# ilovin/lstm_ctc_ocr

Hardware: NVIDIA H100
Metric: text-line images/sec (fwd+CTC loss) (higher is better)
Workload: dtype bf16

## Files before the change

### lstm_ctc_ocr_b200/csrc/lstm.cuh

```cuda
#pragma once
#include <cuda.h>

#include "common.cuh"
#include "wgmma.cuh"

namespace lstm {

constexpr int NUM_THREADS = 384;
constexpr int BLOCK_M = 128;

struct Params {
  const __nv_bfloat16* xproj;
  __nv_bfloat16* h_state;
  __nv_bfloat16* lstm_out;
  const int* seq_len;
  int Nimg, Npad, H, T, tiles_per_dir;
  __nv_bfloat16* gates;
  float* csave;
  int swap_ls;
  long long* trace;
};

#define LSTM_TRACE(ev)                                                                                  \
  do {                                                                                                  \
    if (p.trace != nullptr && lane == 0 && s >= 8 && s < 12 && (blockIdx.x == 0 || blockIdx.x == 5))    \
      p.trace[(((blockIdx.x ? 1 : 0) * 4 + (s - 8)) * 16) + (ev)] = clock64();                          \
  } while (0)

__device__ __forceinline__ uint32_t cluster_ctarank() {
  uint32_t r;
  asm volatile("mov.u32 %0, %%cluster_ctarank;" : "=r"(r));
  return r;
}
__device__ __forceinline__ void cluster_arrive_release() { asm volatile("barrier.cluster.arrive.release.aligned;" ::: "memory"); }
__device__ __forceinline__ void cluster_wait_acquire() { asm volatile("barrier.cluster.wait.acquire.aligned;" ::: "memory"); }
__device__ __forceinline__ void fence_proxy_async_all() { asm volatile("fence.proxy.async;" ::: "memory"); }

template <int CS>
struct Cfg {
  static constexpr int UPC = 256 / CS;
  static constexpr int NCOLS = 4 * UPC;
  static constexpr int B_BYTES = 4 * NCOLS * 128;
  static constexpr int A_BYTES = 4 * BLOCK_M * 128;
  static constexpr int ACC_OFFSET = A_BYTES + B_BYTES;
  static constexpr int BAR_OFFSET = ACC_OFFSET + BLOCK_M * NCOLS * 4;
  static constexpr int SMEM_BYTES = BAR_OFFSET + 128 + 1024;
};

template <int CS>
__global__ void __launch_bounds__(NUM_THREADS, 1)
lstm_persistent_kernel(const __grid_constant__ CUtensorMap tmH, const __grid_constant__ CUtensorMap tmW, const Params p) {
  static_assert(CS == 8, "register budget of the epilogue is sized for 32 units per CTA");
  using C = Cfg<CS>;
  constexpr int UPC = C::UPC, NCOLS = C::NCOLS;
  constexpr int HALF = UPC / 2;

  extern __shared__ uint8_t smem_raw[];
  uint8_t* smem = reinterpret_cast<uint8_t*>((reinterpret_cast<uintptr_t>(smem_raw) + 1023) & ~uintptr_t(1023));
  uint8_t* smem_a = smem;
  uint8_t* smem_b = smem + C::A_BYTES;
  uint64_t* a_full = reinterpret_cast<uint64_t*>(smem + C::BAR_OFFSET);
  uint64_t* b_full = a_full + 4;
  float* acc_tile = reinterpret_cast<float*>(smem + C::ACC_OFFSET);

  const int warp_idx = threadIdx.x >> 5, lane = threadIdx.x & 31;
  const int rank = (int)cluster_ctarank();
  const int unit = blockIdx.x / CS;
  const int dir = unit / p.tiles_per_dir;
  const int tile = unit - dir * p.tiles_per_dir;

  if (warp_idx == 0 && lane == 0) {
    ptx::prefetch_tmap(&tmH);
    ptx::prefetch_tmap(&tmW);
    for (int i = 0; i < 4; ++i) ptx::mbar_init(&a_full[i], 1);
    ptx::mbar_init(b_full, 1);
    ptx::fence_barrier_init();
  }
  __syncthreads();

  if (warp_idx == 0 && lane == 0) {
// ... 98 lines not shown
          if (p.gates != nullptr) {
            const size_t dts = (size_t)unit * p.T + s;
            __nv_bfloat16* gs = p.gates + lstm_gate_off(dts, 0, rank * UPC + u0, row);
            float* cs = p.csave + lstm_c_off(dts, rank * UPC + u0, row);
#pragma unroll
            for (int i = 0; i < HALF; i += 8) {
              *reinterpret_cast<uint4*>(gs + 0 * LSTM_GATE_STRIDE + (i >> 3) * LSTM_GCHUNK_STRIDE) = make_uint4(ptx::pack_bf16x2(__uint_as_float(gi[i]), __uint_as_float(gi[i + 1])), ptx::pack_bf16x2(__uint_as_float(gi[i + 2]), __uint_as_float(gi[i + 3])), ptx::pack_bf16x2(__uint_as_float(gi[i + 4]), __uint_as_float(gi[i + 5])), ptx::pack_bf16x2(__uint_as_float(gi[i + 6]), __uint_as_float(gi[i + 7])));
              *reinterpret_cast<uint4*>(gs + 1 * LSTM_GATE_STRIDE + (i >> 3) * LSTM_GCHUNK_STRIDE) = make_uint4(ptx::pack_bf16x2(__uint_as_float(gj[i]), __uint_as_float(gj[i + 1])), ptx::pack_bf16x2(__uint_as_float(gj[i + 2]), __uint_as_float(gj[i + 3])), ptx::pack_bf16x2(__uint_as_float(gj[i + 4]), __uint_as_float(gj[i + 5])), ptx::pack_bf16x2(__uint_as_float(gj[i + 6]), __uint_as_float(gj[i + 7])));
              *reinterpret_cast<uint4*>(gs + 2 * LSTM_GATE_STRIDE + (i >> 3) * LSTM_GCHUNK_STRIDE) = make_uint4(ptx::pack_bf16x2(__uint_as_float(gf[i]), __uint_as_float(gf[i + 1])), ptx::pack_bf16x2(__uint_as_float(gf[i + 2]), __uint_as_float(gf[i + 3])), ptx::pack_bf16x2(__uint_as_float(gf[i + 4]), __uint_as_float(gf[i + 5])), ptx::pack_bf16x2(__uint_as_float(gf[i + 6]), __uint_as_float(gf[i + 7])));
              *reinterpret_cast<uint4*>(gs + 3 * LSTM_GATE_STRIDE + (i >> 3) * LSTM_GCHUNK_STRIDE) = make_uint4(ptx::pack_bf16x2(__uint_as_float(go[i]), __uint_as_float(go[i + 1])), ptx::pack_bf16x2(__uint_as_float(go[i + 2]), __uint_as_float(go[i + 3])), ptx::pack_bf16x2(__uint_as_float(go[i + 4]), __uint_as_float(go[i + 5])), ptx::pack_bf16x2(__uint_as_float(go[i + 6]), __uint_as_float(go[i + 7])));
            }
#pragma unroll
            for (int i = 0; i < HALF; i += 4)
              *reinterpret_cast<float4*>(cs + (i >> 2) * LSTM_CCHUNK_STRIDE) = make_float4(cst[u0 + i], cst[u0 + i + 1], cst[u0 + i + 2], cst[u0 + i + 3]);
          }
#pragma unroll
          for (int i = 0; i < HALF / 2; ++i) hp[i] = ptx::pack_bf16x2(hv[2 * i], hv[2 * i + 1]);
        } else {
#pragma unroll
          for (int i = 0; i < HALF / 2; ++i) hp[i] = 0u;
        }
        if (okn) {
#pragma unroll
          for (int i = 0; i < HALF / 2; i += 4) {
            const uint4 v = make_uint4(hp[i], hp[i + 1], hp[i + 2], hp[i + 3]);
            *reinterpret_cast<uint4*>(hn + u0 + 2 * i) = v;
            *reinterpret_cast<uint4*>(lo + u0 + 2 * i) = v;
          }
        }
      }
      if (warp_idx == 4) LSTM_TRACE(8);
      fence_proxy_async_all();
      if (warp_idx == 4) LSTM_TRACE(9);
    }
    cluster_arrive_release();
    if (warp_idx == 4) LSTM_TRACE(10);
    cluster_wait_acquire();
    if (warp_idx == 4) LSTM_TRACE(11);
  }
}


template <int EW>
struct McThreads {
  static constexpr int EPI = EW * 32;
  static constexpr int ALL = 128 + EPI;
};

template <int CS>
struct CfgMc {
  static constexpr int UPC = 256 / CS;
  static constexpr int NCOLS = 4 * UPC;
  static constexpr int B_BYTES = 4 * NCOLS * 128;
  static constexpr int A_BYTES = 32 * BLOCK_M * 16;
  static constexpr int SLICE_BYTES = A_BYTES / CS;
  static constexpr int ACC_OFFSET = 2 * A_BYTES + B_BYTES;
  static constexpr int BAR_OFFSET = ACC_OFFSET + BLOCK_M * 64 * 4;
  static constexpr int SMEM_BYTES = BAR_OFFSET + 128 + 1024;
};

__device__ __forceinline__ void bulk_copy_s2s_cluster(uint32_t dst_cluster_addr, const void* src_smem, uint32_t bytes,
                                                      uint32_t bar_cluster_addr) {
  asm volatile("cp.async.bulk.shared::cluster.shared::cta.mbarrier::complete_tx::bytes [%0], [%1], %2, [%3];" ::"r"(dst_cluster_addr),
               "r"(ptx::smem_u32(src_smem)), "r"(bytes), "r"(bar_cluster_addr)
               : "memory");
}

template <int CS, int MODE, int EW>
__global__ void __launch_bounds__(McThreads<EW>::ALL, 1)
lstm_mc_kernel(const __grid_constant__ CUtensorMap tmW, const Params p) {
  static_assert(CS == 8, "8 CTAs x 32 units");
  using C = CfgMc<CS>;
  constexpr int UPC = C::UPC, NCOLS = C::NCOLS;
  constexpr int HALF = UPC / (EW / 4);
  constexpr int MC_EPI_THREADS = McThreads<EW>::EPI;
  static_assert(EW == 8, "epilogue warps = the two MMA warpgroups");
  constexpr bool DS = (MODE == 1), MS = (MODE == 2), GX = (MODE == 3), LOCAL = DS || MS;
  constexpr uint32_t FILL_TX = LOCAL ? (CS - 1) * C::SLICE_BYTES : C::A_BYTES;

  extern __shared__ uint8_t smem_raw[];
  uint8_t* smem = smem_raw + ((1024u - (ptx::smem_u32(smem_raw) & 1023u)) & 1023u);
  uint8_t* smem_a = smem;
  uint8_t* smem_b = smem + 2 * C::A_BYTES;
  uint64_t* a_full = reinterpret_cast<uint64_t*>(smem + C::BAR_OFFSET);
  uint64_t* b_full = a_full + 2;
  uint64_t* part_ready = b_full + 1;
  float* acc_half = reinterpret_cast<float*>(smem + C::ACC_OFFSET);

  const int warp_idx = threadIdx.x >> 5, lane = threadIdx.x & 31;
  const int rank = (int)cluster_ctarank();
  const int unit = blockIdx.x / CS;
  const int dir = unit / p.tiles_per_dir;
  const int tile = unit - dir * p.tiles_per_dir;

  if (warp_idx == 0 && lane == 0) {
    ptx::prefetch_tmap(&tmW);
    ptx::mbar_init(&part_ready[0], CS);
    ptx::mbar_init(&part_ready[1], CS);
    ptx::mbar_init(&a_full[0], GX ? MC_EPI_THREADS : LOCAL ? 2 : 1);
    ptx::mbar_init(&a_full[1], GX ? MC_EPI_THREADS : LOCAL ? 2 : 1);
    ptx::mbar_init(b_full, 1);
    ptx::fence_barrier_init();
    if (!GX && p.T > 1) ptx::mbar_arrive_expect_tx(&a_full[1], FILL_TX);
    if (!GX && p.T > 2) ptx::mbar_arrive_expect_tx(&a_full[0], FILL_TX);
    ptx::mbar_arrive_expect_tx(b_full, C::B_BYTES);
    for (int kb = 0; kb < 4; ++kb)
      ptx::tma_load_2d(&tmW, b_full, smem_b + kb * NCOLS * 128, kb * 64, dir * 1024 + rank * NCOLS);
  }
  __syncthreads();
  cluster_arrive_release();
  cluster_wait_acquire();

  if (warp_idx < 4) {
    ptx::setmaxnreg_dec<40>();
  } else {
    ptx::setmaxnreg_inc<232>();
    const int wgi = (warp_idx >> 2) - 1;
    const int q = warp_idx & 3;
    const int hh = (warp_idx - 4) >> 2;
    const int u0 = hh * HALF;
    const int row = q * 32 + lane;
    const int n = tile * BLOCK_M + row;
    const bool okn = n < p.Nimg;
    const int len = okn ? min(max(__ldg(p.seq_len + n), 0), p.T) : 0;
    float cst[HALF];
#pragma unroll
    for (int i = 0; i < HALF; ++i) cst[i] = 0.f;
    ptx::mbar_wait(b_full, 0);
    const uint32_t slice_off = rank * C::SLICE_BYTES + (u0 / 8) * 2048 + row * 16;
    uint8_t* hx0 = reinterpret_cast<uint8_t*>(p.h_state) + ((size_t)unit * CS + rank) * C::SLICE_BYTES;
    const size_t hx_buf_stride = (size_t)2 * p.tiles_per_dir * CS * C::SLICE_BYTES;

    for (int s = 0; s < p.T; ++s) {
      const bool active = s < len;
      const int t = active ? (dir ? (len - 1 - s) : s) : s;
      uint4 xp[4][HALF / 8];
      if (active) {
        const __nv_bfloat16* src = p.xproj + ((size_t)n * p.H + s) * 2048 + dir * 1024 + rank * NCOLS + u0;
#pragma unroll
        for (int g = 0; g < 4; ++g)
#pragma unroll
          for (int v = 0; v < HALF / 8; ++v) xp[g][v] = __ldg(reinterpret_cast<const uint4*>(src + g * UPC) + v);
      }
      if (warp_idx == 4) LSTM_TRACE(5);
      uint32_t gi[HALF], gj[HALF], gf[HALF], go[HALF];
      if (s > 0) {
        const int b = s & 1;
        ptx::mbar_wait(&a_full[b], ((s - 1) >> 1) & 1);
        if (warp_idx == 4) LSTM_TRACE(3);
        if (!GX && s + 2 < p.T && threadIdx.x == 128) ptx::mbar_arrive_expect_tx(&a_full[b], FILL_TX);
        const uint32_t a_base = ptx::smem_u32(smem_a + b * C::A_BYTES) + wgi * 64 * 16;
        float d[NCOLS / 2];
        wg::fence();
#pragma unroll
        for (int k = 0; k < 16; ++k) {
          const uint64_t a_desc = p.swap_ls ? ptx::make_desc_k_nosw(a_base + k * 4096, 128, 2048) : ptx::make_desc_k_nosw(a_base + k * 4096, 2048, 128);
          const uint64_t b_desc = ptx::make_desc_k_sw128(ptx::smem_u32(smem_b + (k >> 2) * NCOLS * 128)) + 2 * (k & 3);
          wg::mma_bf16<NCOLS>(d, a_desc, b_desc, k != 0);
        }
        wg::commit();
        wg::wait<0>();
        wg::fence_operand(d);
        if (warp_idx == 4) LSTM_TRACE(4);
        const int tt = threadIdx.x & 127, l = tt & 31;
        const int r0 = wgi * 64 + 16 * (tt >> 5) + (l >> 2);
#pragma unroll
        for (int r = 0; r < 2; ++r) {
          ptx::bar_sync(1, MC_EPI_THREADS);
#pragma unroll
          for (int g = 0; g < 4; ++g)
#pragma unroll
            for (int jj = 0; jj < 2; ++jj) {
              const int j = 4 * g + 2 * r + jj;
              const int c = g * 16 + jj * 8 + 2 * (l & 3);
              *reinterpret_cast<float2*>(ptx::acc_chunk<64>(acc_half, r0, c >> 2) + (c & 3)) = make_float2(d[4 * j], d[4 * j + 1]);
              *reinterpret_cast<float2*>(ptx::acc_chunk<64>(acc_half, r0 + 8, c >> 2) + (c & 3)) = make_float2(d[4 * j + 2], d[4 * j + 3]);
            }
          ptx::bar_sync(1, MC_EPI_THREADS);
          if (hh == r) {
            ptx::acc_ld<64, HALF>(acc_half, row, 0, gi);
            ptx::acc_ld<64, HALF>(acc_half, row, 16, gj);
            ptx::acc_ld<64, HALF>(acc_half, row, 32, gf);
            ptx::acc_ld<64, HALF>(acc_half, row, 48, go);
          }
        }
        if (warp_idx == 4) LSTM_TRACE(7);
      } else {
#pragma unroll
        for (int i = 0; i < HALF; ++i) { gi[i] = 0u; gj[i] = 0u; gf[i] = 0u; go[i] = 0u; }
      }
      uint32_t hp[HALF / 2];
      if (active) {
        const uint32_t* xi = reinterpret_cast<const uint32_t*>(xp[0]);
        const uint32_t* xj = reinterpret_cast<const uint32_t*>(xp[1]);
        const uint32_t* xf = reinterpret_cast<const uint32_t*>(xp[2]);
        const uint32_t* xo = reinterpret_cast<const uint32_t*>(xp[3]);
        float hv[HALF];
#pragma unroll
        for (int i = 0; i < HALF; ++i) {
          const float zi = __uint_as_float(gi[i]) + ((i & 1) ? ptx::bf16_hi(xi[i >> 1]) : ptx::bf16_lo(xi[i >> 1]));
          const float zj = __uint_as_float(gj[i]) + ((i & 1) ? ptx::bf16_hi(xj[i >> 1]) : ptx::bf16_lo(xj[i >> 1]));
          const float zf = __uint_as_float(gf[i]) + ((i & 1) ? ptx::bf16_hi(xf[i >> 1]) : ptx::bf16_lo(xf[i >> 1]));
          const float zo = __uint_as_float(go[i]) + ((i & 1) ? ptx::bf16_hi(xo[i >> 1]) : ptx::bf16_lo(xo[i >> 1]));
          const float ai = ptx::fast_sigmoid(zi), aj = ptx::fast_tanh(zj), af = ptx::fast_sigmoid(zf), ao = ptx::fast_sigmoid(zo);
          const float c = af * cst[i] + ai * aj;
          cst[i] = c;
          hv[i] = ao * ptx::fast_tanh(c);
          if (p.gates != nullptr) {
            gi[i] = __float_as_uint(ai); gj[i] = __float_as_uint(aj); gf[i] = __float_as_uint(af); go[i] = __float_as_uint(ao);
          }
        }
#pragma unroll
        for (int i = 0; i < HALF / 2; ++i) hp[i] = ptx::pack_bf16x2(hv[2 * i], hv[2 * i + 1]);
      } else {
#pragma unroll
        for (int i = 0; i < HALF / 2; ++i) hp[i] = 0u;
      }
      if (s + 1 < p.T) {
        const int nb = (s + 1) & 1;
        if (LOCAL) {
          uint8_t* dst = smem_a + nb * C::A_BYTES + slice_off;
#pragma unroll
          for (int v = 0; v < HALF / 8; ++v)
            *reinterpret_cast<uint4*>(dst + v * 2048) = make_uint4(hp[4 * v], hp[4 * v + 1], hp[4 * v + 2], hp[4 * v + 3]);
          ptx::fence_proxy_async_smem();
        } else {
          uint8_t* dst = hx0 + (size_t)nb * hx_buf_stride + (u0 / 8) * 2048 + row * 16;
#pragma unroll
          for (int v = 0; v < HALF / 8; ++v)
            *reinterpret_cast<uint4*>(dst + v * 2048) = make_uint4(hp[4 * v], hp[4 * v + 1], hp[4 * v + 2], hp[4 * v + 3]);
          if (!GX) fence_proxy_async_all();
        }
        if (warp_idx == 4) LSTM_TRACE(8);
        asm volatile("bar.sync 1, %0;" ::"n"(MC_EPI_THREADS) : "memory");
        if (warp_idx == 4) {
          uint8_t* my_slice = smem_a + nb * C::A_BYTES + rank * C::SLICE_BYTES;
          if (DS) {
            if (lane < CS) {
              if (lane == rank) {
                ptx::mbar_arrive(&a_full[nb]);
              } else {
                const uint32_t dst = ptx::mapa(ptx::smem_u32(my_slice), (uint32_t)lane);
                const uint32_t bar = ptx::mapa(ptx::smem_u32(&a_full[nb]), (uint32_t)lane);
                bulk_copy_s2s_cluster(dst, my_slice, C::SLICE_BYTES, bar);
              }
            }
          } else if (MS) {
            if (lane == 0) {
              uint8_t* g = hx0 + (size_t)nb * hx_buf_stride;
              ptx::bulk_store_1d(g, my_slice, C::SLICE_BYTES);
              ptx::bulk_commit();
              asm volatile("cp.async.bulk.wait_group 0;" ::: "memory");
              ptx::bulk_load_1d_mc(my_slice, g, C::SLICE_BYTES, &a_full[nb], (uint16_t)(((1u << CS) - 1) & ~(1u << rank)));
              ptx::mbar_arrive(&a_full[nb]);
            }
          } else if (GX) {
            if (lane < CS) ptx::mbar_arrive_cluster(ptx::mapa(ptx::smem_u32(&part_ready[nb]), (uint32_t)lane));
          } else if (lane == 0) {
            ptx::bulk_load_1d_mc(my_slice, hx0 + (size_t)nb * hx_buf_stride, C::SLICE_BYTES, &a_full[nb], (uint16_t)((1u << CS) - 1));
          }
          __syncwarp();
          LSTM_TRACE(9);
        }
        if (GX) {
          ptx::mbar_wait_cluster(&part_ready[nb], (uint32_t)(s >> 1) & 1u);
          const uint8_t* g = reinterpret_cast<const uint8_t*>(p.h_state) + (size_t)nb * hx_buf_stride + (size_t)unit * CS * C::SLICE_BYTES;
          uint8_t* d = smem_a + nb * C::A_BYTES;
          const int et = threadIdx.x - 128;
          uint4 v[C::A_BYTES / 16 / MC_EPI_THREADS];
#pragma unroll
          for (int k = 0; k < C::A_BYTES / 16 / MC_EPI_THREADS; ++k) v[k] = __ldcg(reinterpret_cast<const uint4*>(g) + k * MC_EPI_THREADS + et);
#pragma unroll
          for (int k = 0; k < C::A_BYTES / 16 / MC_EPI_THREADS; ++k) *(reinterpret_cast<uint4*>(d) + k * MC_EPI_THREADS + et) = v[k];
          ptx::fence_proxy_async_smem();
          ptx::mbar_arrive(&a_full[nb]);
        }
      }
      if (okn) {
        __nv_bfloat16* lo = p.lstm_out + ((size_t)n * p.H + t) * 512 + dir * 256 + rank * UPC + u0;
        if constexpr (HALF == 16) ptx::st_global_v8(lo, hp[0], hp[1], hp[2], hp[3], hp[4], hp[5], hp[6], hp[7]);
        else *reinterpret_cast<uint4*>(lo) = make_uint4(hp[0], hp[1], hp[2], hp[3]);
      }
      if (active && p.gates != nullptr) {
        const size_t dts = (size_t)unit * p.T + s;
        __nv_bfloat16* gs = p.gates + lstm_gate_off(dts, 0, rank * UPC + u0, row);
        float* cs = p.csave + lstm_c_off(dts, rank * UPC + u0, row);
#pragma unroll
        for (int i = 0; i < HALF; i += 8) {
          *reinterpret_cast<uint4*>(gs + 0 * LSTM_GATE_STRIDE + (i >> 3) * LSTM_GCHUNK_STRIDE) = make_uint4(ptx::pack_bf16x2(__uint_as_float(gi[i]), __uint_as_float(gi[i + 1])), ptx::pack_bf16x2(__uint_as_float(gi[i + 2]), __uint_as_float(gi[i + 3])), ptx::pack_bf16x2(__uint_as_float(gi[i + 4]), __uint_as_float(gi[i + 5])), ptx::pack_bf16x2(__uint_as_float(gi[i + 6]), __uint_as_float(gi[i + 7])));
          *reinterpret_cast<uint4*>(gs + 1 * LSTM_GATE_STRIDE + (i >> 3) * LSTM_GCHUNK_STRIDE) = make_uint4(ptx::pack_bf16x2(__uint_as_float(gj[i]), __uint_as_float(gj[i + 1])), ptx::pack_bf16x2(__uint_as_float(gj[i + 2]), __uint_as_float(gj[i + 3])), ptx::pack_bf16x2(__uint_as_float(gj[i + 4]), __uint_as_float(gj[i + 5])), ptx::pack_bf16x2(__uint_as_float(gj[i + 6]), __uint_as_float(gj[i + 7])));
          *reinterpret_cast<uint4*>(gs + 2 * LSTM_GATE_STRIDE + (i >> 3) * LSTM_GCHUNK_STRIDE) = make_uint4(ptx::pack_bf16x2(__uint_as_float(gf[i]), __uint_as_float(gf[i + 1])), ptx::pack_bf16x2(__uint_as_float(gf[i + 2]), __uint_as_float(gf[i + 3])), ptx::pack_bf16x2(__uint_as_float(gf[i + 4]), __uint_as_float(gf[i + 5])), ptx::pack_bf16x2(__uint_as_float(gf[i + 6]), __uint_as_float(gf[i + 7])));
          *reinterpret_cast<uint4*>(gs + 3 * LSTM_GATE_STRIDE + (i >> 3) * LSTM_GCHUNK_STRIDE) = make_uint4(ptx::pack_bf16x2(__uint_as_float(go[i]), __uint_as_float(go[i + 1])), ptx::pack_bf16x2(__uint_as_float(go[i + 2]), __uint_as_float(go[i + 3])), ptx::pack_bf16x2(__uint_as_float(go[i + 4]), __uint_as_float(go[i + 5])), ptx::pack_bf16x2(__uint_as_float(go[i + 6]), __uint_as_float(go[i + 7])));
        }
#pragma unroll
        for (int i = 0; i < HALF; i += 4) *reinterpret_cast<float4*>(cs + (i >> 2) * LSTM_CCHUNK_STRIDE) = make_float4(cst[i], cst[i + 1], cst[i + 2], cst[i + 3]);
      }
      if (warp_idx == 4) LSTM_TRACE(10);
    }
  }

  __syncthreads();
  cluster_arrive_release();
  cluster_wait_acquire();
}

}
```

### lstm_ctc_ocr_b200/csrc/model.cu

```cuda
#include <cstdarg>
#include <cstring>
#include <string>
#include <vector>

#include <cstdlib>
#include <condition_variable>
#include <mutex>
#include <thread>

#include "gemm_launch.h"
#include "lstm.cuh"
#include "conv_swap.cuh"
#include "conv1_tc.cuh"
#include "kernels.cuh"
#include "model_internal.h"

static thread_local char g_err[1024] = "";
int crnn_fail(int status, const char* fmt, ...) {
  va_list ap;
  va_start(ap, fmt);
  vsnprintf(g_err, sizeof(g_err), fmt, ap);
  va_end(ap);
  return status;
}
// ... 565 lines not shown
    float* bn = pl.bn;
    if (m->dp_world > 1)
      CRNN_TRY(dp_allreduce_bn_finalize(m, pl.stats, bn_count * m->dp_world, m->P("conv4_1/conv4_1/gamma"), m->P("conv4_1/conv4_1/beta"),
                                        m->cfg.bn_eps, bn, st));
    else
    CRNN_TRY(launch_bn_finalize(pl.stats, bn_count, m->P("conv4_1/conv4_1/gamma"), m->P("conv4_1/conv4_1/beta"),
                                m->cfg.bn_eps, bn, bn + 512, bn + 1024, bn + 1536, 512, st));
    CRNN_TRY(launch_bn_apply_relu(pl.a4a_pre, pl.a4a, bn, bn + 512, (size_t)N * H2 * 4, 512, st));
  }
  STAGE_MARK();
  {
    gemm::Params p = conv_params(N, H2, 4, 512, 512, 256, m->P("conv4_2/biases"), pl.a4b_pre, pl.mg4);
    p.stats = pl.stats + 1024;
    CRNN_TRY((launch_gemm<256, gemm::A_CONV3, gemm::EPI_STATS, 4>(pl.tA_c42, m->tB_c42, p, sms, st, &pl.tO_c42)));
    STAGE_MARK();
    float* bn = pl.bn + 2048;
    if (m->dp_world > 1)
      CRNN_TRY(dp_allreduce_bn_finalize(m, pl.stats + 1024, bn_count * m->dp_world, m->P("conv4_2/conv4_2/gamma"),
                                        m->P("conv4_2/conv4_2/beta"), m->cfg.bn_eps, bn, st));
    else
    CRNN_TRY(launch_bn_finalize(pl.stats + 1024, bn_count, m->P("conv4_2/conv4_2/gamma"), m->P("conv4_2/conv4_2/beta"),
                                m->cfg.bn_eps, bn, bn + 512, bn + 1024, bn + 1536, 512, st));
    CRNN_TRY(launch_bn_apply_relu_pool12(pl.a4b_pre, pl.a4b, bn, bn + 512, (size_t)N * H2 * 2, 512, st));
  }
  STAGE_MARK();
  {
    gemm::Params p;
    memset(&p, 0, sizeof(p));
    p.M = N * H2;
    p.num_m_tiles = (p.M + 127) / 128; p.num_n_tiles = 2; p.num_k_blocks = 32; p.kb_per_shift = 16; p.row_shift_mul = 1;
    p.Nc = 512; p.bias = m->P("conv5/biases"); p.out = pl.a5; p.ldo = 512;
    CRNN_TRY((launch_gemm<256, gemm::A_PLAIN, gemm::EPI_BIAS_BF16, 4>(pl.tA_c5, m->tB_c5, p, sms, st, &pl.tA_x)));
  }
  STAGE_MARK();
  {
    gemm::Params p;
    memset(&p, 0, sizeof(p));
    p.M = N * H2;
    p.num_m_tiles = (p.M + 127) / 128; p.num_n_tiles = 8; p.num_k_blocks = 8; p.kb_per_shift = 8;
    p.Nc = 2048; p.bias = m->xbias; p.out = pl.xproj; p.ldo = 2048;
    p.H = H2; p.T = T; p.seq_len = time_step_len;
    if (m->lstm_upc == 32) CRNN_TRY((launch_gemm<256, gemm::A_PLAIN, gemm::EPI_XPROJ, 4>(pl.tA_x, m->tB_x, p, sms, st, &pl.tO_x)));
    else CRNN_TRY((launch_gemm<256, gemm::A_PLAIN, gemm::EPI_BIAS_BF16, 4>(pl.tA_x, m->tB_x, p, sms, st, &pl.tO_x)));
  }
  STAGE_MARK();
  if (m->lstm_upc == 32) {
    constexpr int CS = 8;
    lstm::Params lp;
    lp.xproj = pl.xproj; lp.h_state = pl.h_state; lp.lstm_out = pl.lstm_out; lp.seq_len = time_step_len;
    lp.Nimg = N; lp.Npad = pl.Npad; lp.H = H2; lp.T = T; lp.tiles_per_dir = pl.Npad / 128;
    lp.gates = pl.train ? pl.gates : nullptr; lp.csave = pl.train ? pl.csave : nullptr;
    static long long* d_trace = nullptr;
    const bool want_trace = getenv("CRNN_LSTM_TRACE") != nullptr;
    if (want_trace && d_trace == nullptr) CUDA_TRY(cudaMalloc(&d_trace, 2 * 4 * 16 * sizeof(long long)));
    if (want_trace) CUDA_TRY(cudaMemsetAsync(d_trace, 0, 2 * 4 * 16 * sizeof(long long), st));
    lp.trace = want_trace ? d_trace : nullptr;
    lp.swap_ls = getenv("CRNN_LSTM_SWAPLS") != nullptr;
    auto kern = lstm::lstm_persistent_kernel<CS>;
    auto kern_mc = lstm::lstm_mc_kernel<CS, 0, 8>;
    auto kern_ds = lstm::lstm_mc_kernel<CS, 1, 8>;
    auto kern_ms = lstm::lstm_mc_kernel<CS, 2, 8>;
    auto kern_gx = lstm::lstm_mc_kernel<CS, 3, 8>;
    static bool attr = false;
    if (!attr) {
      CUDA_TRY(cudaFuncSetAttribute(kern, cudaFuncAttributeMaxDynamicSharedMemorySize, lstm::Cfg<CS>::SMEM_BYTES));
      CUDA_TRY(cudaFuncSetAttribute(kern_mc, cudaFuncAttributeMaxDynamicSharedMemorySize, lstm::CfgMc<CS>::SMEM_BYTES));
      CUDA_TRY(cudaFuncSetAttribute(kern_ds, cudaFuncAttributeMaxDynamicSharedMemorySize, lstm::CfgMc<CS>::SMEM_BYTES));
      CUDA_TRY(cudaFuncSetAttribute(kern_ms, cudaFuncAttributeMaxDynamicSharedMemorySize, lstm::CfgMc<CS>::SMEM_BYTES));
      CUDA_TRY(cudaFuncSetAttribute(kern_gx, cudaFuncAttributeMaxDynamicSharedMemorySize, lstm::CfgMc<CS>::SMEM_BYTES));
      attr = true;
    }
    cudaLaunchConfig_t cfg;
    memset(&cfg, 0, sizeof(cfg));
    cfg.gridDim = dim3(CS * 2 * lp.tiles_per_dir);
    cfg.blockDim = dim3(m->lstm_mc ? lstm::McThreads<8>::ALL : lstm::NUM_THREADS);
    cfg.dynamicSmemBytes = m->lstm_mc ? lstm::CfgMc<CS>::SMEM_BYTES : lstm::Cfg<CS>::SMEM_BYTES;
    cfg.stream = st;
    cudaLaunchAttribute at[1];
    at[0].id = cudaLaunchAttributeClusterDimension;
    at[0].val.clusterDim.x = CS; at[0].val.clusterDim.y = 1; at[0].val.clusterDim.z = 1;
    cfg.attrs = at; cfg.numAttrs = 1;
    if (m->lstm_mc == 4) CUDA_TRY(cudaLaunchKernelEx(&cfg, kern_gx, m->tB_h128, lp));
    else if (m->lstm_mc == 3) CUDA_TRY(cudaLaunchKernelEx(&cfg, kern_ms, m->tB_h128, lp));
    else if (m->lstm_mc == 2) CUDA_TRY(cudaLaunchKernelEx(&cfg, kern_ds, m->tB_h128, lp));
    else if (m->lstm_mc == 1) CUDA_TRY(cudaLaunchKernelEx(&cfg, kern_mc, m->tB_h128, lp));
    else CUDA_TRY(cudaLaunchKernelEx(&cfg, kern, pl.tA_hall, m->tB_h128, lp));
    if (want_trace) {
      long long h[2 * 4 * 16];
      CUDA_TRY(cudaStreamSynchronize(st));
      CUDA_TRY(cudaMemcpy(h, d_trace, sizeof(h), cudaMemcpyDeviceToHost));
      for (int c = 0; c < 2; ++c)
        for (int s = 0; s < 4; ++s) {
          fprintf(stderr, "lstm_trace cta%d step%d:", c ? 5 : 0, 8 + s);
          for (int e = 0; e < 12; ++e) fprintf(stderr, " %lld", h[(c * 4 + s) * 16 + e] ? h[(c * 4 + s) * 16 + e] - h[(c * 4) * 16] : -1);
          fprintf(stderr, "\n");
        }
    }
  } else {
    CUDA_TRY(cudaMemsetAsync(pl.h_state, 0, (size_t)2 * pl.Npad * 256 * 2, st));
    CUDA_TRY(cudaMemsetAsync(pl.c_state, 0, (size_t)2 * pl.Npad * 256 * 4, st));
    for (int s = 0; s < T; ++s) {
      gemm::Params p;
      memset(&p, 0, sizeof(p));
      p.num_m_tiles = 2 * pl.Npad / 128; p.num_n_tiles = 4; p.num_k_blocks = 4; p.kb_per_shift = 4;
      p.m_tiles_per_dir = pl.Npad / 128;
      p.Nc = 1024; p.H = H2; p.T = T; p.Nimg = N; p.Npad = pl.Npad; p.step = s;
      p.xproj = pl.xproj; p.c_state = pl.c_state; p.lstm_out = pl.lstm_out; p.seq_len = time_step_len;
      p.h_next = pl.h_state + (size_t)((s + 1) & 1) * 2 * pl.Npad * 256;
      CRNN_TRY((launch_gemm<256, gemm::A_PLAIN, gemm::EPI_LSTM, 4>(pl.tA_h[s & 1], m->tB_h, p, sms, st)));
    }
  }
  STAGE_MARK();
  {
    gemm::Params p;
    memset(&p, 0, sizeof(p));
    p.M = N * H2;
    p.num_m_tiles = (p.M + 127) / 128; p.num_n_tiles = 1; p.num_k_blocks = 8; p.kb_per_shift = 8;
    p.Nc = 64; p.bias = m->P("logits/biases"); p.out = logits_out; p.H = H2; p.T = T; p.Nimg = N;
    CRNN_TRY((launch_gemm<64, gemm::A_PLAIN, gemm::EPI_LOGITS, 8>(pl.tA_l, m->tB_l, p, sms, st)));
  }
  STAGE_MARK();
#undef STAGE_MARK
  return CRNN_OK;
}

extern "C" int crnn_forward(crnn_model* m, const float* data, const int* time_step_len, int N, int W, float* logits_out,
                            void* workspace, size_t workspace_bytes, crnn_stream_t stream) {
  cudaStream_t st = reinterpret_cast<cudaStream_t>(stream);
  return forward_impl(m, data, nullptr, time_step_len, N, W, logits_out, workspace, workspace_bytes, 1, st, st);
}

extern "C" int crnn_forward_host(crnn_model* m, const float* host_data, float* data_staging, const int* time_step_len, int N, int W,
                                 float* logits_out, void* workspace, size_t workspace_bytes, int chunks, crnn_stream_t stream,
                                 crnn_stream_t copy_stream) {
  if (!host_data || !data_staging) return crnn_fail(CRNN_INVALID_VALUE, "forward_host: null pointer");
  return forward_impl(m, data_staging, host_data, time_step_len, N, W, logits_out, workspace, workspace_bytes, chunks,
                      reinterpret_cast<cudaStream_t>(stream), reinterpret_cast<cudaStream_t>(copy_stream));
}

extern "C" int crnn_host_copy(void* dst, const void* src, size_t bytes, int threads) {
  if ((!dst || !src) && bytes) return crnn_fail(CRNN_INVALID_VALUE, "host_copy: null pointer");
  CopyPool::get().copy(dst, src, bytes, threads < 1 ? 1 : threads);
  return CRNN_OK;
}

extern "C" int crnn_forward_pageable(crnn_model* m, const float* pageable_data, float* pinned_staging, float* data_staging,
                                     const int* time_step_len, int N, int W, float* logits_out, void* workspace, size_t workspace_bytes,
                                     int chunks, int host_threads, crnn_stream_t stream, crnn_stream_t copy_stream) {
  if (!pageable_data || !pinned_staging || !data_staging) return crnn_fail(CRNN_INVALID_VALUE, "forward_pageable: null pointer");
// ... 139 lines not shown
```

Baseline: 173,200.

## Run LSTM cell math on WGMMA fragments in registers and decouple warpgroup halves

```diff
diff --git a/lstm_ctc_ocr_b200/csrc/lstm.cuh b/lstm_ctc_ocr_b200/csrc/lstm.cuh
--- a/lstm_ctc_ocr_b200/csrc/lstm.cuh
+++ b/lstm_ctc_ocr_b200/csrc/lstm.cuh
@@ -21,11 +21,12 @@
   long long* trace;
 };
 
-#define LSTM_TRACE(ev)                                                                                  \
+#define LSTM_TRACE_WG(wg, ev)                                                                           \
   do {                                                                                                  \
     if (p.trace != nullptr && lane == 0 && s >= 8 && s < 12 && (blockIdx.x == 0 || blockIdx.x == 5))    \
-      p.trace[(((blockIdx.x ? 1 : 0) * 4 + (s - 8)) * 16) + (ev)] = clock64();                          \
+      p.trace[((((blockIdx.x ? 1 : 0) * 2 + (wg)) * 4 + (s - 8)) * 16) + (ev)] = clock64();             \
   } while (0)
+#define LSTM_TRACE(ev) LSTM_TRACE_WG(0, ev)
 
 __device__ __forceinline__ uint32_t cluster_ctarank() {
   uint32_t r;
@@ -230,10 +231,11 @@
   static constexpr int UPC = 256 / CS;
   static constexpr int NCOLS = 4 * UPC;
   static constexpr int B_BYTES = 4 * NCOLS * 128;
-  static constexpr int A_BYTES = 32 * BLOCK_M * 16;
-  static constexpr int SLICE_BYTES = A_BYTES / CS;
-  static constexpr int ACC_OFFSET = 2 * A_BYTES + B_BYTES;
-  static constexpr int BAR_OFFSET = ACC_OFFSET + BLOCK_M * 64 * 4;
+  static constexpr int HALF_ROWS = BLOCK_M / 2;
+  static constexpr int HALF_A_BYTES = 32 * HALF_ROWS * 16;
+  static constexpr int A_BYTES = 2 * HALF_A_BYTES;
+  static constexpr int SLICE_BYTES = HALF_A_BYTES / CS;
+  static constexpr int BAR_OFFSET = 2 * A_BYTES + B_BYTES;
   static constexpr int SMEM_BYTES = BAR_OFFSET + 128 + 1024;
 };
 
@@ -250,20 +252,18 @@
   static_assert(CS == 8, "8 CTAs x 32 units");
   using C = CfgMc<CS>;
   constexpr int UPC = C::UPC, NCOLS = C::NCOLS;
-  constexpr int HALF = UPC / (EW / 4);
-  constexpr int MC_EPI_THREADS = McThreads<EW>::EPI;
   static_assert(EW == 8, "epilogue warps = the two MMA warpgroups");
+  static_assert(NCOLS == 128, "fragment column group j = gate j/4, units 8(j%4) ..: one m64n128 product per half and step");
   constexpr bool DS = (MODE == 1), MS = (MODE == 2), GX = (MODE == 3), LOCAL = DS || MS;
-  constexpr uint32_t FILL_TX = LOCAL ? (CS - 1) * C::SLICE_BYTES : C::A_BYTES;
+  constexpr uint32_t FILL_TX = LOCAL ? (CS - 1) * C::SLICE_BYTES : C::HALF_A_BYTES;
 
   extern __shared__ uint8_t smem_raw[];
   uint8_t* smem = smem_raw + ((1024u - (ptx::smem_u32(smem_raw) & 1023u)) & 1023u);
   uint8_t* smem_a = smem;
   uint8_t* smem_b = smem + 2 * C::A_BYTES;
   uint64_t* a_full = reinterpret_cast<uint64_t*>(smem + C::BAR_OFFSET);
-  uint64_t* b_full = a_full + 2;
+  uint64_t* b_full = a_full + 4;
   uint64_t* part_ready = b_full + 1;
-  float* acc_half = reinterpret_cast<float*>(smem + C::ACC_OFFSET);
 
   const int warp_idx = threadIdx.x >> 5, lane = threadIdx.x & 31;
   const int rank = (int)cluster_ctarank();
@@ -273,14 +273,16 @@
 
   if (warp_idx == 0 && lane == 0) {
     ptx::prefetch_tmap(&tmW);
-    ptx::mbar_init(&part_ready[0], CS);
-    ptx::mbar_init(&part_ready[1], CS);
-    ptx::mbar_init(&a_full[0], GX ? MC_EPI_THREADS : LOCAL ? 2 : 1);
-    ptx::mbar_init(&a_full[1], GX ? MC_EPI_THREADS : LOCAL ? 2 : 1);
+    for (int i = 0; i < 4; ++i) {
+      ptx::mbar_init(&part_ready[i], CS);
+      ptx::mbar_init(&a_full[i], GX ? 128 : LOCAL ? 2 : 1);
+    }
     ptx::mbar_init(b_full, 1);
     ptx::fence_barrier_init();
-    if (!GX && p.T > 1) ptx::mbar_arrive_expect_tx(&a_full[1], FILL_TX);
-    if (!GX && p.T > 2) ptx::mbar_arrive_expect_tx(&a_full[0], FILL_TX);
+    for (int hf = 0; hf < 2; ++hf) {
+      if (!GX && p.T > 1) ptx::mbar_arrive_expect_tx(&a_full[2 * hf + 1], FILL_TX);
+      if (!GX && p.T > 2) ptx::mbar_arrive_expect_tx(&a_full[2 * hf + 0], FILL_TX);
+    }
     ptx::mbar_arrive_expect_tx(b_full, C::B_BYTES);
     for (int kb = 0; kb < 4; ++kb)
       ptx::tma_load_2d(&tmW, b_full, smem_b + kb * NCOLS * 128, kb * 64, dir * 1024 + rank * NCOLS);
@@ -294,186 +296,182 @@
   } else {
     ptx::setmaxnreg_inc<232>();
     const int wgi = (warp_idx >> 2) - 1;
-    const int q = warp_idx & 3;
-    const int hh = (warp_idx - 4) >> 2;
-    const int u0 = hh * HALF;
-    const int row = q * 32 + lane;
-    const int n = tile * BLOCK_M + row;
-    const bool okn = n < p.Nimg;
-    const int len = okn ? min(max(__ldg(p.seq_len + n), 0), p.T) : 0;
-    float cst[HALF];
-#pragma unroll
-    for (int i = 0; i < HALF; ++i) cst[i] = 0.f;
+    const int w = warp_idx & 3, q4 = lane & 3;
+    const int rr0 = 16 * w + (lane >> 2);
+    int n[2], len[2];
+    bool okn[2];
+#pragma unroll
+    for (int rh = 0; rh < 2; ++rh) {
+      n[rh] = tile * BLOCK_M + wgi * C::HALF_ROWS + rr0 + 8 * rh;
+      okn[rh] = n[rh] < p.Nimg;
+      len[rh] = okn[rh] ? min(max(__ldg(p.seq_len + n[rh]), 0), p.T) : 0;
+    }
+    float cst[2][4][2];
+#pragma unroll
+    for (int rh = 0; rh < 2; ++rh)
+#pragma unroll
+      for (int k = 0; k < 4; ++k) { cst[rh][k][0] = 0.f; cst[rh][k][1] = 0.f; }
+    uint64_t* my_full = a_full + 2 * wgi;
+    uint64_t* my_ready = part_ready + 2 * wgi;
     ptx::mbar_wait(b_full, 0);
-    const uint32_t slice_off = rank * C::SLICE_BYTES + (u0 / 8) * 2048 + row * 16;
-    uint8_t* hx0 = reinterpret_cast<uint8_t*>(p.h_state) + ((size_t)unit * CS + rank) * C::SLICE_BYTES;
-    const size_t hx_buf_stride = (size_t)2 * p.tiles_per_dir * CS * C::SLICE_BYTES;
+    const uint32_t word_off = rr0 * 16 + q4 * 4;
+    uint8_t* hx_half = reinterpret_cast<uint8_t*>(p.h_state) + (size_t)(unit * 2 + wgi) * C::HALF_A_BYTES;
+    const size_t hx_buf_stride = (size_t)2 * p.tiles_per_dir * C::A_BYTES;
 
     for (int s = 0; s < p.T; ++s) {
-      const bool active = s < len;
-      const int t = active ? (dir ? (len - 1 - s) : s) : s;
-      uint4 xp[4][HALF / 8];
-      if (active) {
-        const __nv_bfloat16* src = p.xproj + ((size_t)n * p.H + s) * 2048 + dir * 1024 + rank * NCOLS + u0;
-#pragma unroll
-        for (int g = 0; g < 4; ++g)
-#pragma unroll
-          for (int v = 0; v < HALF / 8; ++v) xp[g][v] = __ldg(reinterpret_cast<const uint4*>(src + g * UPC) + v);
-      }
-      if (warp_idx == 4) LSTM_TRACE(5);
-      uint32_t gi[HALF], gj[HALF], gf[HALF], go[HALF];
+      bool active[2];
+      int t[2];
+      uint32_t xw[2][4][4];
+#pragma unroll
+      for (int rh = 0; rh < 2; ++rh) {
+        active[rh] = s < len[rh];
+        t[rh] = active[rh] ? (dir ? (len[rh] - 1 - s) : s) : s;
+        if (active[rh]) {
+          const uint32_t* src = reinterpret_cast<const uint32_t*>(p.xproj + ((size_t)n[rh] * p.H + s) * 2048 + dir * 1024 + rank * NCOLS + 2 * q4);
+#pragma unroll
+          for (int g = 0; g < 4; ++g)
+#pragma unroll
+            for (int k = 0; k < 4; ++k) xw[rh][g][k] = __ldg(src + (g * UPC + 8 * k) / 2);
+        } else {
+#pragma unroll
+          for (int g = 0; g < 4; ++g)
+#pragma unroll
+            for (int k = 0; k < 4; ++k) xw[rh][g][k] = 0u;
+        }
+      }
+      if (q4 < 2) {
+#pragma unroll
+        for (int rh = 0; rh < 2; ++rh)
+          if (s + 1 < len[rh])
+            asm volatile("prefetch.global.L2 [%0];" ::"l"(p.xproj + ((size_t)n[rh] * p.H + s + 1) * 2048 + dir * 1024 + rank * NCOLS + q4 * 64));
+      }
+      if (w == 0) LSTM_TRACE_WG(wgi, 5);
+      float d[NCOLS / 2];
       if (s > 0) {
         const int b = s & 1;
-        ptx::mbar_wait(&a_full[b], ((s - 1) >> 1) & 1);
-        if (warp_idx == 4) LSTM_TRACE(3);
-        if (!GX && s + 2 < p.T && threadIdx.x == 128) ptx::mbar_arrive_expect_tx(&a_full[b], FILL_TX);
-        const uint32_t a_base = ptx::smem_u32(smem_a + b * C::A_BYTES) + wgi * 64 * 16;
-        float d[NCOLS / 2];
+        ptx::mbar_wait(&my_full[b], ((s - 1) >> 1) & 1);
+        if (w == 0) LSTM_TRACE_WG(wgi, 3);
+        if (!GX && s + 2 < p.T && (threadIdx.x & 127) == 0) ptx::mbar_arrive_expect_tx(&my_full[b], FILL_TX);
+        const uint32_t a_base = ptx::smem_u32(smem_a + b * C::A_BYTES + wgi * C::HALF_A_BYTES);
         wg::fence();
 #pragma unroll
         for (int k = 0; k < 16; ++k) {
-          const uint64_t a_desc = p.swap_ls ? ptx::make_desc_k_nosw(a_base + k * 4096, 128, 2048) : ptx::make_desc_k_nosw(a_base + k * 4096, 2048, 128);
+          const uint64_t a_desc = p.swap_ls ? ptx::make_desc_k_nosw(a_base + k * 2048, 128, 1024) : ptx::make_desc_k_nosw(a_base + k * 2048, 1024, 128);
           const uint64_t b_desc = ptx::make_desc_k_sw128(ptx::smem_u32(smem_b + (k >> 2) * NCOLS * 128)) + 2 * (k & 3);
           wg::mma_bf16<NCOLS>(d, a_desc, b_desc, k != 0);
         }
         wg::commit();
         wg::wait<0>();
         wg::fence_operand(d);
-        if (warp_idx == 4) LSTM_TRACE(4);
-        const int tt = threadIdx.x & 127, l = tt & 31;
-        const int r0 = wgi * 64 + 16 * (tt >> 5) + (l >> 2);
-#pragma unroll
-        for (int r = 0; r < 2; ++r) {
-          ptx::bar_sync(1, MC_EPI_THREADS);
-#pragma unroll
-          for (int g = 0; g < 4; ++g)
-#pragma unroll
-            for (int jj = 0; jj < 2; ++jj) {
-              const int j = 4 * g + 2 * r + jj;
-              const int c = g * 16 + jj * 8 + 2 * (l & 3);
-              *reinterpret_cast<float2*>(ptx::acc_chunk<64>(acc_half, r0, c >> 2) + (c & 3)) = make_float2(d[4 * j], d[4 * j + 1]);
-              *reinterpret_cast<float2*>(ptx::acc_chunk<64>(acc_half, r0 + 8, c >> 2) + (c & 3)) = make_float2(d[4 * j + 2], d[4 * j + 3]);
+        if (w == 0) LSTM_TRACE_WG(wgi, 4);
+      } else {
+#pragma unroll
+        for (int i = 0; i < NCOLS / 2; ++i) d[i] = 0.f;
+      }
+      uint32_t hw[2][4];
+#pragma unroll
+      for (int rh = 0; rh < 2; ++rh)
+#pragma unroll
+        for (int k = 0; k < 4; ++k) {
+          hw[rh][k] = 0u;
+          if (active[rh]) {
+            float hv[2];
+#pragma unroll
+            for (int e = 0; e < 2; ++e) {
+              const int f = 4 * k + 2 * rh + e;
+              const float zi = d[f] + (e ? ptx::bf16_hi(xw[rh][0][k]) : ptx::bf16_lo(xw[rh][0][k]));
+              const float zj = d[16 + f] + (e ? ptx::bf16_hi(xw[rh][1][k]) : ptx::bf16_lo(xw[rh][1][k]));
+              const float zf = d[32 + f] + (e ? ptx::bf16_hi(xw[rh][2][k]) : ptx::bf16_lo(xw[rh][2][k]));
+              const float zo = d[48 + f] + (e ? ptx::bf16_hi(xw[rh][3][k]) : ptx::bf16_lo(xw[rh][3][k]));
+              const float ai = ptx::fast_sigmoid(zi), aj = ptx::fast_tanh(zj), af = ptx::fast_sigmoid(zf), ao = ptx::fast_sigmoid(zo);
+              const float c = af * cst[rh][k][e] + ai * aj;
+              cst[rh][k][e] = c;
+              hv[e] = ao * ptx::fast_tanh(c);
+              d[f] = ai; d[16 + f] = aj; d[32 + f] = af; d[48 + f] = ao;
             }
-          ptx::bar_sync(1, MC_EPI_THREADS);
-          if (hh == r) {
-            ptx::acc_ld<64, HALF>(acc_half, row, 0, gi);
-            ptx::acc_ld<64, HALF>(acc_half, row, 16, gj);
-            ptx::acc_ld<64, HALF>(acc_half, row, 32, gf);
-            ptx::acc_ld<64, HALF>(acc_half, row, 48, go);
+            hw[rh][k] = ptx::pack_bf16x2(hv[0], hv[1]);
           }
         }
-        if (warp_idx == 4) LSTM_TRACE(7);
-      } else {
-#pragma unroll
-        for (int i = 0; i < HALF; ++i) { gi[i] = 0u; gj[i] = 0u; gf[i] = 0u; go[i] = 0u; }
-      }
-      uint32_t hp[HALF / 2];
-      if (active) {
-        const uint32_t* xi = reinterpret_cast<const uint32_t*>(xp[0]);
-        const uint32_t* xj = reinterpret_cast<const uint32_t*>(xp[1]);
-        const uint32_t* xf = reinterpret_cast<const uint32_t*>(xp[2]);
-        const uint32_t* xo = reinterpret_cast<const uint32_t*>(xp[3]);
-        float hv[HALF];
-#pragma unroll
-        for (int i = 0; i < HALF; ++i) {
-          const float zi = __uint_as_float(gi[i]) + ((i & 1) ? ptx::bf16_hi(xi[i >> 1]) : ptx::bf16_lo(xi[i >> 1]));
-          const float zj = __uint_as_float(gj[i]) + ((i & 1) ? ptx::bf16_hi(xj[i >> 1]) : ptx::bf16_lo(xj[i >> 1]));
-          const float zf = __uint_as_float(gf[i]) + ((i & 1) ? ptx::bf16_hi(xf[i >> 1]) : ptx::bf16_lo(xf[i >> 1]));
-          const float zo = __uint_as_float(go[i]) + ((i & 1) ? ptx::bf16_hi(xo[i >> 1]) : ptx::bf16_lo(xo[i >> 1]));
-          const float ai = ptx::fast_sigmoid(zi), aj = ptx::fast_tanh(zj), af = ptx::fast_sigmoid(zf), ao = ptx::fast_sigmoid(zo);
-          const float c = af * cst[i] + ai * aj;
-          cst[i] = c;
-          hv[i] = ao * ptx::fast_tanh(c);
-          if (p.gates != nullptr) {
-            gi[i] = __float_as_uint(ai); gj[i] = __float_as_uint(aj); gf[i] = __float_as_uint(af); go[i] = __float_as_uint(ao);
-          }
-        }
-#pragma unroll
-        for (int i = 0; i < HALF / 2; ++i) hp[i] = ptx::pack_bf16x2(hv[2 * i], hv[2 * i + 1]);
-      } else {
-#pragma unroll
-        for (int i = 0; i < HALF / 2; ++i) hp[i] = 0u;
-      }
+      if (w == 0) LSTM_TRACE_WG(wgi, 7);
       if (s + 1 < p.T) {
         const int nb = (s + 1) & 1;
-        if (LOCAL) {
-          uint8_t* dst = smem_a + nb * C::A_BYTES + slice_off;
-#pragma unroll
-          for (int v = 0; v < HALF / 8; ++v)
-            *reinterpret_cast<uint4*>(dst + v * 2048) = make_uint4(hp[4 * v], hp[4 * v + 1], hp[4 * v + 2], hp[4 * v + 3]);
-          ptx::fence_proxy_async_smem();
-        } else {
-          uint8_t* dst = hx0 + (size_t)nb * hx_buf_stride + (u0 / 8) * 2048 + row * 16;
-#pragma unroll
-          for (int v = 0; v < HALF / 8; ++v)
-            *reinterpret_cast<uint4*>(dst + v * 2048) = make_uint4(hp[4 * v], hp[4 * v + 1], hp[4 * v + 2], hp[4 * v + 3]);
-          if (!GX) fence_proxy_async_all();
-        }
-        if (warp_idx == 4) LSTM_TRACE(8);
-        asm volatile("bar.sync 1, %0;" ::"n"(MC_EPI_THREADS) : "memory");
-        if (warp_idx == 4) {
-          uint8_t* my_slice = smem_a + nb * C::A_BYTES + rank * C::SLICE_BYTES;
+        uint8_t* my_slice = smem_a + nb * C::A_BYTES + wgi * C::HALF_A_BYTES + rank * C::SLICE_BYTES;
+        uint8_t* hx_slice = hx_half + (size_t)nb * hx_buf_stride + rank * C::SLICE_BYTES;
+        uint8_t* dst = (LOCAL ? my_slice : hx_slice) + word_off;
+#pragma unroll
+        for (int rh = 0; rh < 2; ++rh)
+#pragma unroll
+          for (int k = 0; k < 4; ++k) *reinterpret_cast<uint32_t*>(dst + k * 1024 + rh * 128) = hw[rh][k];
+        if (LOCAL) ptx::fence_proxy_async_smem();
+        else if (!GX) fence_proxy_async_all();
+        if (w == 0) LSTM_TRACE_WG(wgi, 8);
+        if (wgi == 0) ptx::bar_sync(1, 128);
+        else ptx::bar_sync(2, 128);
+        if (w == 0) {
           if (DS) {
             if (lane < CS) {
               if (lane == rank) {
-                ptx::mbar_arrive(&a_full[nb]);
+                ptx::mbar_arrive(&my_full[nb]);
               } else {
-                const uint32_t dst = ptx::mapa(ptx::smem_u32(my_slice), (uint32_t)lane);
-                const uint32_t bar = ptx::mapa(ptx::smem_u32(&a_full[nb]), (uint32_t)lane);
-                bulk_copy_s2s_cluster(dst, my_slice, C::SLICE_BYTES, bar);
+                const uint32_t dst_peer = ptx::mapa(ptx::smem_u32(my_slice), (uint32_t)lane);
+                const uint32_t bar = ptx::mapa(ptx::smem_u32(&my_full[nb]), (uint32_t)lane);
+                bulk_copy_s2s_cluster(dst_peer, my_slice, C::SLICE_BYTES, bar);
               }
             }
           } else if (MS) {
             if (lane == 0) {
-              uint8_t* g = hx0 + (size_t)nb * hx_buf_stride;
-              ptx::bulk_store_1d(g, my_slice, C::SLICE_BYTES);
+              ptx::bulk_store_1d(hx_slice, my_slice, C::SLICE_BYTES);
               ptx::bulk_commit();
               asm volatile("cp.async.bulk.wait_group 0;" ::: "memory");
-              ptx::bulk_load_1d_mc(my_slice, g, C::SLICE_BYTES, &a_full[nb], (uint16_t)(((1u << CS) - 1) & ~(1u << rank)));
-              ptx::mbar_arrive(&a_full[nb]);
+              ptx::bulk_load_1d_mc(my_slice, hx_slice, C::SLICE_BYTES, &my_full[nb], (uint16_t)(((1u << CS) - 1) & ~(1u << rank)));
+              ptx::mbar_arrive(&my_full[nb]);
             }
           } else if (GX) {
-            if (lane < CS) ptx::mbar_arrive_cluster(ptx::mapa(ptx::smem_u32(&part_ready[nb]), (uint32_t)lane));
+            if (lane < CS) ptx::mbar_arrive_cluster(ptx::mapa(ptx::smem_u32(&my_ready[nb]), (uint32_t)lane));
           } else if (lane == 0) {
-            ptx::bulk_load_1d_mc(my_slice, hx0 + (size_t)nb * hx_buf_stride, C::SLICE_BYTES, &a_full[nb], (uint16_t)((1u << CS) - 1));
+            ptx::bulk_load_1d_mc(my_slice, hx_slice, C::SLICE_BYTES, &my_full[nb], (uint16_t)((1u << CS) - 1));
           }
           __syncwarp();
-          LSTM_TRACE(9);
+          LSTM_TRACE_WG(wgi, 9);
         }
         if (GX) {
-          ptx::mbar_wait_cluster(&part_ready[nb], (uint32_t)(s >> 1) & 1u);
-          const uint8_t* g = reinterpret_cast<const uint8_t*>(p.h_state) + (size_t)nb * hx_buf_stride + (size_t)unit * CS * C::SLICE_BYTES;
-          uint8_t* d = smem_a + nb * C::A_BYTES;
-          const int et = threadIdx.x - 128;
-          uint4 v[C::A_BYTES / 16 / MC_EPI_THREADS];
-#pragma unroll
-          for (int k = 0; k < C::A_BYTES / 16 / MC_EPI_THREADS; ++k) v[k] = __ldcg(reinterpret_cast<const uint4*>(g) + k * MC_EPI_THREADS + et);
-#pragma unroll
-          for (int k = 0; k < C::A_BYTES / 16 / MC_EPI_THREADS; ++k) *(reinterpret_cast<uint4*>(d) + k * MC_EPI_THREADS + et) = v[k];
+          ptx::mbar_wait_cluster(&my_ready[nb], (uint32_t)(s >> 1) & 1u);
+          const uint8_t* g = hx_half + (size_t)nb * hx_buf_stride;
+          uint8_t* a = smem_a + nb * C::A_BYTES + wgi * C::HALF_A_BYTES;
+          const int et = threadIdx.x & 127;
+          uint4 v[C::HALF_A_BYTES / 16 / 128];
+#pragma unroll
+          for (int k = 0; k < C::HALF_A_BYTES / 16 / 128; ++k) v[k] = __ldcg(reinterpret_cast<const uint4*>(g) + k * 128 + et);
+#pragma unroll
+          for (int k = 0; k < C::HALF_A_BYTES / 16 / 128; ++k) *(reinterpret_cast<uint4*>(a) + k * 128 + et) = v[k];
           ptx::fence_proxy_async_smem();
-          ptx::mbar_arrive(&a_full[nb]);
-        }
-      }
-      if (okn) {
-        __nv_bfloat16* lo = p.lstm_out + ((size_t)n * p.H + t) * 512 + dir * 256 + rank * UPC + u0;
-        if constexpr (HALF == 16) ptx::st_global_v8(lo, hp[0], hp[1], hp[2], hp[3], hp[4], hp[5], hp[6], hp[7]);
-        else *reinterpret_cast<uint4*>(lo) = make_uint4(hp[0], hp[1], hp[2], hp[3]);
-      }
-      if (active && p.gates != nullptr) {
-        const size_t dts = (size_t)unit * p.T + s;
-        __nv_bfloat16* gs = p.gates + lstm_gate_off(dts, 0, rank * UPC + u0, row);
-        float* cs = p.csave + lstm_c_off(dts, rank * UPC + u0, row);
-#pragma unroll
-        for (int i = 0; i < HALF; i += 8) {
-          *reinterpret_cast<uint4*>(gs + 0 * LSTM_GATE_STRIDE + (i >> 3) * LSTM_GCHUNK_STRIDE) = make_uint4(ptx::pack_bf16x2(__uint_as_float(gi[i]), __uint_as_float(gi[i + 1])), ptx::pack_bf16x2(__uint_as_float(gi[i + 2]), __uint_as_float(gi[i + 3])), ptx::pack_bf16x2(__uint_as_float(gi[i + 4]), __uint_as_float(gi[i + 5])), ptx::pack_bf16x2(__uint_as_float(gi[i + 6]), __uint_as_float(gi[i + 7])));
-          *reinterpret_cast<uint4*>(gs + 1 * LSTM_GATE_STRIDE + (i >> 3) * LSTM_GCHUNK_STRIDE) = make_uint4(ptx::pack_bf16x2(__uint_as_float(gj[i]), __uint_as_float(gj[i + 1])), ptx::pack_bf16x2(__uint_as_float(gj[i + 2]), __uint_as_float(gj[i + 3])), ptx::pack_bf16x2(__uint_as_float(gj[i + 4]), __uint_as_float(gj[i + 5])), ptx::pack_bf16x2(__uint_as_float(gj[i + 6]), __uint_as_float(gj[i + 7])));
-          *reinterpret_cast<uint4*>(gs + 2 * LSTM_GATE_STRIDE + (i >> 3) * LSTM_GCHUNK_STRIDE) = make_uint4(ptx::pack_bf16x2(__uint_as_float(gf[i]), __uint_as_float(gf[i + 1])), ptx::pack_bf16x2(__uint_as_float(gf[i + 2]), __uint_as_float(gf[i + 3])), ptx::pack_bf16x2(__uint_as_float(gf[i + 4]), __uint_as_float(gf[i + 5])), ptx::pack_bf16x2(__uint_as_float(gf[i + 6]), __uint_as_float(gf[i + 7])));
-          *reinterpret_cast<uint4*>(gs + 3 * LSTM_GATE_STRIDE + (i >> 3) * LSTM_GCHUNK_STRIDE) = make_uint4(ptx::pack_bf16x2(__uint_as_float(go[i]), __uint_as_float(go[i + 1])), ptx::pack_bf16x2(__uint_as_float(go[i + 2]), __uint_as_float(go[i + 3])), ptx::pack_bf16x2(__uint_as_float(go[i + 4]), __uint_as_float(go[i + 5])), ptx::pack_bf16x2(__uint_as_float(go[i + 6]), __uint_as_float(go[i + 7])));
-        }
-#pragma unroll
-        for (int i = 0; i < HALF; i += 4) *reinterpret_cast<float4*>(cs + (i >> 2) * LSTM_CCHUNK_STRIDE) = make_float4(cst[i], cst[i + 1], cst[i + 2], cst[i + 3]);
-      }
-      if (warp_idx == 4) LSTM_TRACE(10);
+          ptx::mbar_arrive(&my_full[nb]);
+        }
+      }
+#pragma unroll
+      for (int rh = 0; rh < 2; ++rh) {
+        if (okn[rh]) {
+          __nv_bfloat16* lo = p.lstm_out + ((size_t)n[rh] * p.H + t[rh]) * 512 + dir * 256 + rank * UPC + 2 * q4;
+#pragma unroll
+          for (int k = 0; k < 4; ++k) *reinterpret_cast<uint32_t*>(lo + 8 * k) = hw[rh][k];
+        }
+        if (active[rh] && p.gates != nullptr) {
+          const size_t dts = (size_t)unit * p.T + s;
+          const int row = wgi * C::HALF_ROWS + rr0 + 8 * rh;
+          __nv_bfloat16* gs = p.gates + lstm_gate_off(dts, 0, rank * UPC, row) + 2 * q4;
+          float* cs = p.csave + lstm_c_off(dts, rank * UPC, row) + 2 * (q4 & 1);
+#pragma unroll
+          for (int g = 0; g < 4; ++g)
+#pragma unroll
+            for (int k = 0; k < 4; ++k)
+              *reinterpret_cast<uint32_t*>(gs + g * LSTM_GATE_STRIDE + k * LSTM_GCHUNK_STRIDE) =
+                  ptx::pack_bf16x2(d[16 * g + 4 * k + 2 * rh], d[16 * g + 4 * k + 2 * rh + 1]);
+#pragma unroll
+          for (int k = 0; k < 4; ++k)
+            *reinterpret_cast<float2*>(cs + (2 * k + (q4 >> 1)) * LSTM_CCHUNK_STRIDE) = make_float2(cst[rh][k][0], cst[rh][k][1]);
+        }
+      }
+      if (w == 0) LSTM_TRACE_WG(wgi, 10);
     }
   }
 
diff --git a/lstm_ctc_ocr_b200/csrc/model.cu b/lstm_ctc_ocr_b200/csrc/model.cu
--- a/lstm_ctc_ocr_b200/csrc/model.cu
+++ b/lstm_ctc_ocr_b200/csrc/model.cu
@@ -641,8 +641,8 @@
     lp.gates = pl.train ? pl.gates : nullptr; lp.csave = pl.train ? pl.csave : nullptr;
     static long long* d_trace = nullptr;
     const bool want_trace = getenv("CRNN_LSTM_TRACE") != nullptr;
-    if (want_trace && d_trace == nullptr) CUDA_TRY(cudaMalloc(&d_trace, 2 * 4 * 16 * sizeof(long long)));
-    if (want_trace) CUDA_TRY(cudaMemsetAsync(d_trace, 0, 2 * 4 * 16 * sizeof(long long), st));
+    if (want_trace && d_trace == nullptr) CUDA_TRY(cudaMalloc(&d_trace, 2 * 2 * 4 * 16 * sizeof(long long)));
+    if (want_trace) CUDA_TRY(cudaMemsetAsync(d_trace, 0, 2 * 2 * 4 * 16 * sizeof(long long), st));
     lp.trace = want_trace ? d_trace : nullptr;
     lp.swap_ls = getenv("CRNN_LSTM_SWAPLS") != nullptr;
     auto kern = lstm::lstm_persistent_kernel<CS>;
@@ -675,15 +675,24 @@
     else if (m->lstm_mc == 1) CUDA_TRY(cudaLaunchKernelEx(&cfg, kern_mc, m->tB_h128, lp));
     else CUDA_TRY(cudaLaunchKernelEx(&cfg, kern, pl.tA_hall, m->tB_h128, lp));
     if (want_trace) {
-      long long h[2 * 4 * 16];
+      long long h[2 * 2 * 4 * 16];
       CUDA_TRY(cudaStreamSynchronize(st));
       CUDA_TRY(cudaMemcpy(h, d_trace, sizeof(h), cudaMemcpyDeviceToHost));
-      for (int c = 0; c < 2; ++c)
-        for (int s = 0; s < 4; ++s) {
-          fprintf(stderr, "lstm_trace cta%d step%d:", c ? 5 : 0, 8 + s);
-          for (int e = 0; e < 12; ++e) fprintf(stderr, " %lld", h[(c * 4 + s) * 16 + e] ? h[(c * 4 + s) * 16 + e] - h[(c * 4) * 16] : -1);
-          fprintf(stderr, "\n");
-        }
+      for (int c = 0; c < 2; ++c) {
+        long long t0 = 0;
+        for (int i = c * 128; i < (c + 1) * 128; ++i)
+          if (h[i] && (!t0 || h[i] < t0)) t0 = h[i];
+        for (int wg = 0; wg < 2; ++wg)
+          for (int s = 0; s < 4; ++s) {
+            const long long* r = h + ((c * 2 + wg) * 4 + s) * 16;
+            bool any = false;
+            for (int e = 0; e < 16; ++e) any = any || r[e];
+            if (!any) continue;
+            fprintf(stderr, "lstm_trace cta%d wg%d step%d:", c ? 5 : 0, wg, 8 + s);
+            for (int e = 0; e < 12; ++e) fprintf(stderr, " %lld", r[e] ? r[e] - t0 : -1);
+            fprintf(stderr, "\n");
+          }
+      }
     }
   } else {
     CUDA_TRY(cudaMemsetAsync(pl.h_state, 0, (size_t)2 * pl.Npad * 256 * 2, st));
```

After: 179,200 (median of 6 runs). 1.04x the previous value.
